# Wodlfvllf/QuintNet

Hardware: AMD Instinct MI355X
Metric: samples/sec (higher is better)
Workload: dtype bf16; 1 GPU; model=gpt2-124M, global_batch=32, seq_len=1024, micro_batch=32, grad_acc=1, parallelism=dp1_tp1_pp1, optimizer=zero1-adamw

## Files before the change

quintnet_amd/csrc/bindings.cpp:

```cpp
#include <torch/extension.h>
#include <ATen/cuda/CUDAContext.h>
#include <hip/hip_runtime.h>

#include <vector>

template <typename T>
void layernorm_fwd_launch(const T*, const T*, const T*, const T*, T*, T*, float*, float*, int, int, float, hipStream_t);
template <typename T>
void layernorm_bwd_launch(const T*, const T*, const T*, const float*, const float*, const T*, T*, float*, float*, int, int, hipStream_t);
int layernorm_bwd_chunks(int rows);
template <typename T>
void softmax_fwd_launch(const T*, T*, long long, int, int, float, int, hipStream_t);
template <typename T>
void softmax_bwd_launch(const T*, const T*, T*, long long, int, float, hipStream_t);
template <typename T>
void ce_fwd_launch(const T*, const long long*, float*, float*, long long, int, long long, hipStream_t);
template <typename T>
void ce_bwd_launch(const T*, const long long*, const float*, const float*, const long long*, T*, long long, int, long long, float, hipStream_t);
template <typename T>
void act_bwd_launch(const T*, const T*, T*, long long, int, hipStream_t);
template <typename T>
void colsum_launch(const T*, float*, long long, int, hipStream_t);
long long colsum_bf16_chunks(long long rows, int N);
int wgrad_tn_splits(int M, int N, int K);
void wgrad_tn_launch(const unsigned short*, const unsigned short*, float*,
                     unsigned short*, int, int, int, int, hipStream_t);
bool colsum_bf16_launch(const unsigned short*, float*, unsigned short*,
                        long long, int, hipStream_t);
template <typename T>
void dropout_fwd_launch(const T*, T*, unsigned char*, long long, float, unsigned, hipStream_t);
template <typename T>
void dropout_bwd_launch(const T*, T*, const unsigned char*, long long, float, hipStream_t);
template <typename T>
void embedding_pair_fwd_launch(const long long*, const T*, const T*, T*, long long, int, int, hipStream_t);
template <typename T>
void embedding_pair_bwd_launch(const long long*, const long long*, const T*, float*, float*, float*, long long, long long, int, int, hipStream_t);
long long embedding_bwd_chunks(long long rows);
template <typename TP, typename TG>
void adamw_launch(TP*, float*, const TG*, float*, float*, const long long*, long long, float, float, float, float, float, int, hipStream_t);
template <typename T>
void sumsq_launch(const T*, long long, float*, hipStream_t);
long long sumsq_blocks(long long n);
std::vector<at::Tensor> gemm_bias_gelu_aux(at::Tensor x, at::Tensor w,
                                           at::Tensor bias);
void gemm_nt_launch(const unsigned short*, const unsigned short*, const unsigned short*,
                    unsigned short*, unsigned short*, int, int, int, int, hipStream_t,
                    int mode = 0);
struct AttnStrides {
  long long qB, qH, qT, kB, kH, kT, vB, vH, vT, oB, oH, oT;
};
void attn_fwd_launch(const unsigned short*, const unsigned short*, const unsigned short*,
                     unsigned short*, float*, int, int, int, int, int, float,
                     int, const AttnStrides&, hipStream_t);
void attn_delta_launch(const unsigned short*, const unsigned short*, float*, int, int, int,
                       long long, long long, long long, long long, long long, long long,
                       hipStream_t);
void attn_bwd_dq_launch(const unsigned short*, const unsigned short*, const unsigned short*,
                        const unsigned short*, const float*, const float*, unsigned short*,
                        int, int, int, int, int, float, int, const AttnStrides&,
                        long long, long long, long long, hipStream_t);
void attn_bwd_dkv_launch(const unsigned short*, const unsigned short*, const unsigned short*,
                         const unsigned short*, const float*, const float*, unsigned short*,
                         unsigned short*, int, int, int, int, int, float, int, const AttnStrides&,
                         long long, long long, long long, long long, long long, long long,
                         long long, long long, long long, hipStream_t);

namespace {

hipStream_t cur_stream() {
  return (hipStream_t)at::cuda::getCurrentCUDAStream().stream();
}

const unsigned short* bf16p(const torch::Tensor& t) {
  return reinterpret_cast<const unsigned short*>(t.data_ptr<at::BFloat16>());
}
unsigned short* bf16p_mut(torch::Tensor& t) {
  return reinterpret_cast<unsigned short*>(t.data_ptr<at::BFloat16>());
}

#define CHECK_GPU(t) TORCH_CHECK(t.is_cuda(), #t " must be on GPU")

std::vector<torch::Tensor> gemm_nt(torch::Tensor x, torch::Tensor w,
                                   c10::optional<torch::Tensor> bias, int64_t act,
                                   int64_t mode) {
  CHECK_GPU(x); CHECK_GPU(w);
  TORCH_CHECK(x.dtype() == torch::kBFloat16 && w.dtype() == torch::kBFloat16,
              "gemm_nt: bf16 only");
  TORCH_CHECK(x.dim() == 2 && w.dim() == 2 && x.size(1) == w.size(1),
              "gemm_nt: shape mismatch");
  TORCH_CHECK(x.size(1) % 8 == 0, "gemm_nt: K must be a multiple of 8");
  auto xc = x.contiguous();
  auto wc = w.contiguous();
  int64_t M = xc.size(0), K = xc.size(1), N = wc.size(0);
  auto out = torch::empty({M, N}, xc.options());
  torch::Tensor pre;
  unsigned short* prep = nullptr;
  if (act != 0) {
    pre = torch::empty({M, N}, xc.options());
    prep = bf16p_mut(pre);
  }
  const unsigned short* bp = nullptr;
  torch::Tensor bc;
  if (bias.has_value() && bias->defined()) {
    bc = bias->contiguous();
    TORCH_CHECK(bc.dtype() == torch::kBFloat16, "bias must be bf16");
    bp = bf16p(bc);
  }
  gemm_nt_launch(bf16p(xc), bf16p(wc), bp, bf16p_mut(out), prep,
                 (int)M, (int)N, (int)K, (int)act, cur_stream(), (int)mode);
  if (act != 0) return {out, pre};
  return {out};
}

std::vector<torch::Tensor> layernorm_fwd(torch::Tensor x, torch::Tensor w,
                                         torch::Tensor b, double eps,
                                         c10::optional<torch::Tensor> residual) {
  CHECK_GPU(x);
  auto xc = x.contiguous();
  int64_t H = xc.size(-1);
  int64_t rows = xc.numel() / H;
  auto y = torch::empty_like(xc);
  auto mean = torch::empty({rows}, xc.options().dtype(torch::kFloat32));
  auto rstd = torch::empty({rows}, xc.options().dtype(torch::kFloat32));
  auto wc = w.contiguous(); auto bc = b.contiguous();
  torch::Tensor rc, sum_out;
  bool has_res = residual.has_value() && residual->defined();
  if (has_res) {
    rc = residual->contiguous();
    sum_out = torch::empty_like(xc);
  }
  if (xc.dtype() == torch::kBFloat16) {
    layernorm_fwd_launch<unsigned short>(
        bf16p(xc), has_res ? bf16p(rc) : nullptr, bf16p(wc), bf16p(bc),
        bf16p_mut(y), has_res ? bf16p_mut(sum_out) : nullptr,
        mean.data_ptr<float>(), rstd.data_ptr<float>(), (int)rows, (int)H,
        (float)eps, cur_stream());
  } else {
    layernorm_fwd_launch<float>(
        xc.data_ptr<float>(), has_res ? rc.data_ptr<float>() : nullptr,
        wc.data_ptr<float>(), bc.data_ptr<float>(), y.data_ptr<float>(),
        has_res ? sum_out.data_ptr<float>() : nullptr, mean.data_ptr<float>(),
        rstd.data_ptr<float>(), (int)rows, (int)H, (float)eps, cur_stream());
  }
  if (has_res) return {y, mean, rstd, sum_out};
  return {y, mean, rstd};
}

std::vector<torch::Tensor> layernorm_bwd(torch::Tensor dy, torch::Tensor x,
                                         torch::Tensor w, torch::Tensor mean,
                                         torch::Tensor rstd,
                                         c10::optional<torch::Tensor> dsum) {
  CHECK_GPU(x);
  auto dyc = dy.contiguous(); auto xc = x.contiguous(); auto wc = w.contiguous();
  int64_t H = xc.size(-1);
  int64_t rows = xc.numel() / H;
  auto dx = torch::empty_like(xc);
  int64_t chunks = layernorm_bwd_chunks((int)rows);
  auto part = torch::empty({2, chunks, H}, xc.options().dtype(torch::kFloat32));
  float* dwp = part.data_ptr<float>();
  float* dbp = dwp + chunks * H;
  torch::Tensor dsc;
  bool has_ds = dsum.has_value() && dsum->defined();
  if (has_ds) dsc = dsum->contiguous();
  if (xc.dtype() == torch::kBFloat16) {
    layernorm_bwd_launch<unsigned short>(
        bf16p(dyc), bf16p(xc), bf16p(wc), mean.data_ptr<float>(),
        rstd.data_ptr<float>(), has_ds ? bf16p(dsc) : nullptr, bf16p_mut(dx),
        dwp, dbp, (int)rows, (int)H, cur_stream());
  } else {
    layernorm_bwd_launch<float>(
        dyc.data_ptr<float>(), xc.data_ptr<float>(), wc.data_ptr<float>(),
        mean.data_ptr<float>(), rstd.data_ptr<float>(),
        has_ds ? dsc.data_ptr<float>() : nullptr, dx.data_ptr<float>(),
        dwp, dbp, (int)rows, (int)H, cur_stream());
  }
  auto dwdb = part.sum(1).to(w.dtype());
  return {dx, dwdb[0], dwdb[1]};
}

torch::Tensor softmax_fwd(torch::Tensor scores, double scale, bool causal) {
  CHECK_GPU(scores);
  auto sc = scores.contiguous();
  int64_t S = sc.size(-1);
  int64_t Tq = sc.size(-2);
  long long rows = sc.numel() / S;
  auto out = torch::empty_like(sc);
  if (sc.dtype() == torch::kBFloat16) {
    softmax_fwd_launch<unsigned short>(bf16p(sc), bf16p_mut(out), rows, (int)Tq,
                                       (int)S, (float)scale, causal ? 1 : 0,
                                       cur_stream());
  } else {
    softmax_fwd_launch<float>(sc.data_ptr<float>(), out.data_ptr<float>(), rows,
                              (int)Tq, (int)S, (float)scale, causal ? 1 : 0,
                              cur_stream());
  }
  return out;
}

torch::Tensor softmax_bwd(torch::Tensor p, torch::Tensor dp, double scale) {
  CHECK_GPU(p);
  auto pc = p.contiguous(); auto dpc = dp.contiguous();
  int64_t S = pc.size(-1);
  long long rows = pc.numel() / S;
  auto ds = torch::empty_like(pc);
  if (pc.dtype() == torch::kBFloat16) {
    softmax_bwd_launch<unsigned short>(bf16p(pc), bf16p(dpc), bf16p_mut(ds), rows,
                                       (int)S, (float)scale, cur_stream());
  } else {
    softmax_bwd_launch<float>(pc.data_ptr<float>(), dpc.data_ptr<float>(),
                              ds.data_ptr<float>(), rows, (int)S, (float)scale,
                              cur_stream());
  }
  return ds;
}

std::vector<torch::Tensor> cross_entropy_fwd(torch::Tensor logits,
                                             torch::Tensor target,
                                             int64_t ignore_index) {
  CHECK_GPU(logits);
  auto lc = logits.contiguous();
  auto tc = target.contiguous();
  TORCH_CHECK(tc.dtype() == torch::kInt64, "target must be int64");
  int64_t V = lc.size(-1);
  long long rows = lc.numel() / V;
  auto lse = torch::empty({(int64_t)rows}, lc.options().dtype(torch::kFloat32));
  auto row_loss = torch::empty({(int64_t)rows}, lc.options().dtype(torch::kFloat32));
  if (lc.dtype() == torch::kBFloat16) {
    ce_fwd_launch<unsigned short>(bf16p(lc), (const long long*)tc.data_ptr<int64_t>(),
                                  lse.data_ptr<float>(), row_loss.data_ptr<float>(),
                                  rows, (int)V, ignore_index, cur_stream());
  } else {
    ce_fwd_launch<float>(lc.data_ptr<float>(), (const long long*)tc.data_ptr<int64_t>(),
                         lse.data_ptr<float>(), row_loss.data_ptr<float>(), rows,
                         (int)V, ignore_index, cur_stream());
  }
  auto loss_sum = row_loss.sum();
  auto n_valid = (tc != ignore_index).sum();
  return {loss_sum, n_valid, lse};
}

torch::Tensor cross_entropy_bwd(torch::Tensor logits, torch::Tensor target,
                                torch::Tensor lse, torch::Tensor n_valid,
                                int64_t ignore_index,
                                c10::optional<torch::Tensor> grad_scale) {
  CHECK_GPU(logits);
  auto lc = logits.contiguous();
  auto tc = target.contiguous();
  int64_t V = lc.size(-1);
  long long rows = lc.numel() / V;
  auto dl = torch::empty_like(lc);
  auto nv = n_valid.to(torch::kInt64).contiguous();
  TORCH_CHECK(nv.is_cuda() && nv.numel() == 1, "n_valid must be a GPU scalar");
  const long long* nvp = (const long long*)nv.data_ptr<int64_t>();
  float inv_n = 1.0f;
  const float* gp = nullptr;
  torch::Tensor gs;
  if (grad_scale.has_value() && grad_scale->defined()) {
    gs = grad_scale->to(torch::kFloat32).contiguous();
    TORCH_CHECK(gs.numel() == 1, "grad_scale must be a scalar tensor");
    gp = gs.data_ptr<float>();
  }
  if (lc.dtype() == torch::kBFloat16) {
    ce_bwd_launch<unsigned short>(bf16p(lc), (const long long*)tc.data_ptr<int64_t>(),
                                  lse.data_ptr<float>(), gp, nvp, bf16p_mut(dl),
                                  rows, (int)V, ignore_index, inv_n, cur_stream());
  } else {
    ce_bwd_launch<float>(lc.data_ptr<float>(), (const long long*)tc.data_ptr<int64_t>(),
                         lse.data_ptr<float>(), gp, nvp, dl.data_ptr<float>(),
                         rows, (int)V, ignore_index, inv_n, cur_stream());
  }
  return dl;
}

torch::Tensor embedding_pair_fwd(torch::Tensor ids, torch::Tensor wte,
                                 torch::Tensor wpe) {
  CHECK_GPU(ids);
  auto ic = ids.contiguous();
  TORCH_CHECK(ic.dtype() == torch::kInt64, "ids must be int64");
  int64_t Tlen = ic.size(-1);
  long long rows = ic.numel();
  int64_t H = wte.size(1);
  auto out = torch::empty({ic.size(0), Tlen, H}, wte.options());
  if (wte.dtype() == torch::kBFloat16)
    embedding_pair_fwd_launch<unsigned short>(
        (const long long*)ic.data_ptr<int64_t>(), bf16p(wte), bf16p(wpe),
        bf16p_mut(out), rows, (int)Tlen, (int)H, cur_stream());
  else
    embedding_pair_fwd_launch<float>(
        (const long long*)ic.data_ptr<int64_t>(), wte.data_ptr<float>(),
        wpe.data_ptr<float>(), out.data_ptr<float>(), rows, (int)Tlen, (int)H,
        cur_stream());
  return out;
}

std::vector<torch::Tensor> embedding_pair_bwd(torch::Tensor ids, torch::Tensor dout,
                                              int64_t vocab, int64_t n_pos) {
  CHECK_GPU(ids);
  auto ic = ids.contiguous();
  auto dc = dout.contiguous();
  int64_t Tlen = ic.size(-1);
  long long rows = ic.numel();
  int64_t H = dc.size(-1);
  auto dwte = torch::zeros({vocab, H}, dc.options().dtype(torch::kFloat32));
  auto dwpe = torch::zeros({n_pos, H}, dc.options().dtype(torch::kFloat32));
  TORCH_CHECK(n_pos >= Tlen, "sequence longer than the position table");
  TORCH_CHECK(dc.numel() == rows * H, "dout does not match ids");
  auto sorted = ic.reshape({-1}).sort(true, 0, false);
  auto sid = std::get<0>(sorted).contiguous();
  auto perm = std::get<1>(sorted).contiguous();
  auto part = torch::empty({(int64_t)embedding_bwd_chunks(rows), 2, H},
                           dc.options().dtype(torch::kFloat32));
  if (dc.dtype() == torch::kBFloat16)
    embedding_pair_bwd_launch<unsigned short>(
        (const long long*)sid.data_ptr<int64_t>(),
        (const long long*)perm.data_ptr<int64_t>(), bf16p(dc),
        dwte.data_ptr<float>(), dwpe.data_ptr<float>(), part.data_ptr<float>(),
        rows, (long long)vocab,
        (int)Tlen, (int)H, cur_stream());
  else
    embedding_pair_bwd_launch<float>(
        (const long long*)sid.data_ptr<int64_t>(),
        (const long long*)perm.data_ptr<int64_t>(), dc.data_ptr<float>(),
        dwte.data_ptr<float>(), dwpe.data_ptr<float>(), part.data_ptr<float>(),
        rows, (long long)vocab,
        (int)Tlen, (int)H, cur_stream());
  return {dwte.to(dout.dtype()), dwpe.to(dout.dtype())};
}

std::vector<torch::Tensor> dropout_fwd(torch::Tensor x, double p, int64_t seed) {
  CHECK_GPU(x);
  auto xc = x.contiguous();
  auto y = torch::empty_like(xc);
  auto mask = torch::empty({xc.numel()}, xc.options().dtype(torch::kUInt8));
  if (xc.dtype() == torch::kBFloat16)
    dropout_fwd_launch<unsigned short>(bf16p(xc), bf16p_mut(y), mask.data_ptr<unsigned char>(),
                                       xc.numel(), (float)p, (unsigned)seed, cur_stream());
  else
    dropout_fwd_launch<float>(xc.data_ptr<float>(), y.data_ptr<float>(), mask.data_ptr<unsigned char>(),
                              xc.numel(), (float)p, (unsigned)seed, cur_stream());
  return {y, mask};
}

torch::Tensor dropout_bwd(torch::Tensor dy, torch::Tensor mask, double p) {
  CHECK_GPU(dy);
  auto dyc = dy.contiguous();
  auto dx = torch::empty_like(dyc);
  if (dyc.dtype() == torch::kBFloat16)
    dropout_bwd_launch<unsigned short>(bf16p(dyc), bf16p_mut(dx), mask.data_ptr<unsigned char>(),
                                       dyc.numel(), (float)p, cur_stream());
  else
    dropout_bwd_launch<float>(dyc.data_ptr<float>(), dx.data_ptr<float>(), mask.data_ptr<unsigned char>(),
                              dyc.numel(), (float)p, cur_stream());
  return dx;
}

torch::Tensor wgrad_tn(torch::Tensor dy, torch::Tensor x) {
  CHECK_GPU(dy); CHECK_GPU(x);
  TORCH_CHECK(dy.dtype() == torch::kBFloat16 && x.dtype() == torch::kBFloat16,
              "wgrad_tn: bf16 only");
  auto dyc = dy.contiguous(); auto xc = x.contiguous();
  TORCH_CHECK(dyc.dim() == 2 && xc.dim() == 2 && dyc.size(0) == xc.size(0),
              "wgrad_tn: [M,N],[M,K] expected");
  int64_t M = dyc.size(0), N = dyc.size(1), K = xc.size(1);
  TORCH_CHECK(N % 128 == 0 && K % 128 == 0 && M % 64 == 0,
              "wgrad_tn: shape not eligible");
  int splits = wgrad_tn_splits((int)M, (int)N, (int)K);
  auto slab = torch::empty({splits, N, K}, dyc.options().dtype(torch::kFloat32));
  auto out = torch::empty({N, K}, dyc.options());
  wgrad_tn_launch(bf16p(dyc), bf16p(xc), slab.data_ptr<float>(), bf16p_mut(out),
                  (int)M, (int)N, (int)K, splits, cur_stream());
  return out;
}

torch::Tensor colsum(torch::Tensor x) {
  CHECK_GPU(x);
  auto xc = x.contiguous();
  int64_t N = xc.size(-1);
  long long rows = xc.numel() / N;
  if (xc.dtype() == torch::kBFloat16 && (N & 7) == 0) {
    long long chunks = colsum_bf16_chunks(rows, (int)N);
    auto part = torch::empty({chunks, N}, xc.options().dtype(torch::kFloat32));
    auto out = torch::empty({N}, xc.options());
    if (colsum_bf16_launch(bf16p(xc), part.data_ptr<float>(), bf16p_mut(out),
                           rows, (int)N, cur_stream()))
      return out;
  }
  auto out = torch::zeros({N}, xc.options().dtype(torch::kFloat32));
  if (xc.dtype() == torch::kBFloat16)
    colsum_launch<unsigned short>(bf16p(xc), out.data_ptr<float>(), rows, (int)N, cur_stream());
  else
    colsum_launch<float>(xc.data_ptr<float>(), out.data_ptr<float>(), rows, (int)N, cur_stream());
  return out.to(x.dtype());
}

torch::Tensor act_bwd(torch::Tensor dy, torch::Tensor pre, int64_t act) {
  CHECK_GPU(dy);
  auto dyc = dy.contiguous();
  auto prec = pre.contiguous();
  TORCH_CHECK(dyc.numel() == prec.numel(), "act_bwd size mismatch");
  auto dx = torch::empty_like(dyc);
  if (dyc.dtype() == torch::kBFloat16)
    act_bwd_launch<unsigned short>(bf16p(dyc), bf16p(prec), bf16p_mut(dx),
                                   dyc.numel(), (int)act, cur_stream());
  else
    act_bwd_launch<float>(dyc.data_ptr<float>(), prec.data_ptr<float>(),
                          dx.data_ptr<float>(), dyc.numel(), (int)act, cur_stream());
  return dx;
}

void adamw_step(torch::Tensor param, torch::Tensor master, torch::Tensor grad,
                torch::Tensor m, torch::Tensor v, int64_t step, double lr,
                double beta1, double beta2, double eps, double wd,
                c10::optional<torch::Tensor> step_dev) {
  CHECK_GPU(param);
  long long n = param.numel();
  TORCH_CHECK(master.numel() == n && grad.numel() == n && m.numel() == n && v.numel() == n,
              "adamw_step: size mismatch");
  auto st = cur_stream();
  float* mp = master.data_ptr<float>();
  float* m1 = m.data_ptr<float>();
  float* m2 = v.data_ptr<float>();
  const long long* sd = nullptr;
  if (step_dev.has_value() && step_dev->defined())
    sd = (const long long*)step_dev->data_ptr<int64_t>();
  bool pbf = param.dtype() == torch::kBFloat16;
  bool gbf = grad.dtype() == torch::kBFloat16;
  if (pbf && gbf)
    adamw_launch<unsigned short, unsigned short>(bf16p_mut(param), mp, bf16p(grad), m1, m2, sd, n,
        (float)lr, (float)beta1, (float)beta2, (float)eps, (float)wd, (int)step, st);
  else if (pbf && !gbf)
    adamw_launch<unsigned short, float>(bf16p_mut(param), mp, grad.data_ptr<float>(), m1, m2, sd, n,
        (float)lr, (float)beta1, (float)beta2, (float)eps, (float)wd, (int)step, st);
  else if (!pbf && gbf)
    adamw_launch<float, unsigned short>(param.data_ptr<float>(), mp, bf16p(grad), m1, m2, sd, n,
        (float)lr, (float)beta1, (float)beta2, (float)eps, (float)wd, (int)step, st);
  else
    adamw_launch<float, float>(param.data_ptr<float>(), mp, grad.data_ptr<float>(), m1, m2, sd, n,
        (float)lr, (float)beta1, (float)beta2, (float)eps, (float)wd, (int)step, st);
}

torch::Tensor multi_tensor_sumsq(std::vector<torch::Tensor> tensors) {
  TORCH_CHECK(!tensors.empty(), "empty tensor list");
  int64_t total = 0;
  for (auto& t : tensors) total += sumsq_blocks(t.numel());
  auto part = torch::empty({total}, tensors[0].options().dtype(torch::kFloat32));
  auto st = cur_stream();
  int64_t off = 0;
  for (auto& t : tensors) {
    auto tc = t.contiguous();
    float* pp = part.data_ptr<float>() + off;
    if (tc.dtype() == torch::kBFloat16)
      sumsq_launch<unsigned short>(bf16p(tc), tc.numel(), pp, st);
    else
      sumsq_launch<float>(tc.data_ptr<float>(), tc.numel(), pp, st);
    off += sumsq_blocks(tc.numel());
  }
  return part.sum();
}


namespace {
void check_attn_view(const torch::Tensor& t, int64_t B, int64_t H, int64_t T) {
  TORCH_CHECK(t.dim() == 4 && t.size(0) == B && t.size(1) == H && t.size(2) == T &&
              t.size(3) == 64, "attn: bad view shape");
  TORCH_CHECK(t.stride(3) == 1, "attn: head_dim must be contiguous");
  TORCH_CHECK(t.stride(2) % 8 == 0 && t.stride(1) % 8 == 0 && t.stride(0) % 8 == 0,
              "attn: strides must be 16B-aligned");
  TORCH_CHECK(t.dtype() == torch::kBFloat16, "attn: bf16 only");
}
const unsigned short* ap(const torch::Tensor& t) {
  return reinterpret_cast<const unsigned short*>(t.data_ptr<at::BFloat16>());
}
unsigned short* ap_mut(torch::Tensor& t) {
  return reinterpret_cast<unsigned short*>(t.data_ptr<at::BFloat16>());
}
}

torch::Tensor attn_fwd(torch::Tensor q, torch::Tensor k, torch::Tensor v,
                       torch::Tensor out, double scale, bool causal,
                       int64_t q_offset) {
  int64_t B = q.size(0), H = q.size(1), Tq = q.size(2), Tk = k.size(2);
  TORCH_CHECK(Tq % 128 == 0 && Tk % 128 == 0 && q_offset % 128 == 0,
              "attn: Tq/Tk/q_offset must be multiples of 128");
  TORCH_CHECK(q_offset >= 0 && q_offset + Tq <= Tk,
              "attn: q rows [q_offset, q_offset+Tq) must lie within [0, Tk)");
  check_attn_view(q, B, H, Tq); check_attn_view(k, B, H, Tk);
  check_attn_view(v, B, H, Tk); check_attn_view(out, B, H, Tq);
  auto lse2 = torch::empty({B * H, Tq}, q.options().dtype(torch::kFloat32));
  AttnStrides st{q.stride(0), q.stride(1), q.stride(2), k.stride(0), k.stride(1),
                 k.stride(2), v.stride(0), v.stride(1), v.stride(2), out.stride(0),
                 out.stride(1), out.stride(2)};
  attn_fwd_launch(ap(q), ap(k), ap(v), ap_mut(out), lse2.data_ptr<float>(),
                  (int)B, (int)H, (int)Tq, (int)Tk, (int)q_offset, (float)scale,
                  causal ? 1 : 0, st, cur_stream());
  return lse2;
}

void attn_bwd(torch::Tensor q, torch::Tensor k, torch::Tensor v,
              torch::Tensor out, torch::Tensor dout, torch::Tensor lse2,
              torch::Tensor dq, torch::Tensor dk, torch::Tensor dv,
              double scale, bool causal, int64_t q_offset) {
  int64_t B = q.size(0), H = q.size(1), Tq = q.size(2), Tk = k.size(2);
  check_attn_view(dout, B, H, Tq); check_attn_view(dq, B, H, Tq);
  check_attn_view(dk, B, H, Tk); check_attn_view(dv, B, H, Tk);
  auto delta = torch::empty({B * H, Tq}, q.options().dtype(torch::kFloat32));
  attn_delta_launch(ap(dout), ap(out), delta.data_ptr<float>(), (int)B, (int)H,
                    (int)Tq, dout.stride(0), dout.stride(1), dout.stride(2),
                    out.stride(0), out.stride(1), out.stride(2), cur_stream());
  AttnStrides st{q.stride(0), q.stride(1), q.stride(2), k.stride(0), k.stride(1),
                 k.stride(2), v.stride(0), v.stride(1), v.stride(2), dq.stride(0),
                 dq.stride(1), dq.stride(2)};
  attn_bwd_dq_launch(ap(q), ap(k), ap(v), ap(dout), lse2.data_ptr<float>(),
                     delta.data_ptr<float>(), ap_mut(dq), (int)B, (int)H,
                     (int)Tq, (int)Tk, (int)q_offset,
                     (float)scale, causal ? 1 : 0, st, dout.stride(0),
                     dout.stride(1), dout.stride(2), cur_stream());
  attn_bwd_dkv_launch(ap(q), ap(k), ap(v), ap(dout), lse2.data_ptr<float>(),
                      delta.data_ptr<float>(), ap_mut(dk), ap_mut(dv), (int)B,
                      (int)H, (int)Tq, (int)Tk, (int)q_offset, (float)scale,
                      causal ? 1 : 0, st,
                      dout.stride(0), dout.stride(1), dout.stride(2),
                      dk.stride(0), dk.stride(1), dk.stride(2), dv.stride(0),
                      dv.stride(1), dv.stride(2), cur_stream());
}

}

PYBIND11_MODULE(TORCH_EXTENSION_NAME, m) {
  m.def("gemm_nt", &gemm_nt, "bf16 MFMA NT GEMM with fused bias/activation",
        py::arg("x"), py::arg("w"), py::arg("bias") = c10::nullopt,
        py::arg("act") = 0, py::arg("mode") = 0);
  m.def("layernorm_fwd", &layernorm_fwd);
  m.def("layernorm_bwd", &layernorm_bwd);
  m.def("softmax_fwd", &softmax_fwd);
  m.def("softmax_bwd", &softmax_bwd);
  m.def("cross_entropy_fwd", &cross_entropy_fwd);
  m.def("cross_entropy_bwd", &cross_entropy_bwd);
  m.def("act_bwd", &act_bwd, "fused activation backward");
  m.def("colsum", &colsum, "column sum (bias grad)");
  m.def("wgrad_tn", &wgrad_tn, "split-K TN weight gradient (tr-read MFMA)");
  m.def("dropout_fwd", &dropout_fwd);
  m.def("embedding_pair_fwd", &embedding_pair_fwd);
  m.def("embedding_pair_bwd", &embedding_pair_bwd);
  m.def("dropout_bwd", &dropout_bwd);
  m.def("attn_fwd", &attn_fwd, "fused flash attention forward (D=64)",
        py::arg("q"), py::arg("k"), py::arg("v"), py::arg("out"),
        py::arg("scale"), py::arg("causal"), py::arg("q_offset") = 0);
  m.def("attn_bwd", &attn_bwd, "fused flash attention backward (D=64)",
        py::arg("q"), py::arg("k"), py::arg("v"), py::arg("out"),
        py::arg("dout"), py::arg("lse2"), py::arg("dq"), py::arg("dk"),
        py::arg("dv"), py::arg("scale"), py::arg("causal"),
        py::arg("q_offset") = 0);
  m.def("adamw_step", &adamw_step);
  m.def("gemm_bias_gelu_aux", &gemm_bias_gelu_aux,
        "hipBLASLt GEMM + fused bias/GELU epilogue (aux = pre-activation)");
  m.def("multi_tensor_sumsq", &multi_tensor_sumsq);
  m.attr("gfx") = "gfx950";
}
```

quintnet_amd/csrc/layernorm.hip:

```cpp
#include "common.h"

template <typename T, int WPB>
__global__ void layernorm_fwd_kernel(
    const T* __restrict__ x, const T* __restrict__ res,
    const T* __restrict__ w, const T* __restrict__ b,
    T* __restrict__ y, T* __restrict__ sum_out,
    float* __restrict__ mean_out, float* __restrict__ rstd_out,
    int rows, int H, float eps) {
  const int lane = threadIdx.x & (QN_WAVE - 1);
  const int wave = threadIdx.x / QN_WAVE;
  const long long row = (long long)blockIdx.x * WPB + wave;
  if (row >= rows) return;
  const T* xr = x + row * H;
  const T* rr = res ? res + row * H : nullptr;
  T* yr = y + row * H;
  T* sr = sum_out ? sum_out + row * H : nullptr;

  float sum = 0.f, sq = 0.f;
  float cache[16];
  const bool cached = H <= QN_WAVE * 16;
  const bool vec8 = sizeof(T) == 2 && (H & 7) == 0 && H >= 512;
  if (cached && vec8) {
    int n = 0;
    for (int i = lane * 8; i < H; i += QN_WAVE * 8, n += 8) {
      ld8_f32(reinterpret_cast<const unsigned short*>(xr) + i, cache + n);
      if (rr) {
        float rv[8];
        ld8_f32(reinterpret_cast<const unsigned short*>(rr) + i, rv);
#pragma unroll
        for (int j = 0; j < 8; ++j) cache[n + j] += rv[j];
        if (sr) st8_f32(reinterpret_cast<unsigned short*>(sr) + i, cache + n);
      }
#pragma unroll
      for (int j = 0; j < 8; ++j) {
        sum += cache[n + j];
        sq += cache[n + j] * cache[n + j];
      }
    }
  } else if (cached) {
    int n = 0;
    for (int i = lane; i < H; i += QN_WAVE, ++n) {
      float f = ld_as_f32(xr + i);
      if (rr) {
        f += ld_as_f32(rr + i);
        if (sr) st_from_f32(sr + i, f);
      }
      cache[n] = f;
      sum += f; sq += f * f;
    }
  } else {
    for (int i = lane; i < H; i += QN_WAVE) {
      float f = ld_as_f32(xr + i);
      if (rr) {
        f += ld_as_f32(rr + i);
        if (sr) st_from_f32(sr + i, f);
      }
      sum += f; sq += f * f;
    }
  }
  sum = wave_reduce_sum(sum);
  sq = wave_reduce_sum(sq);
  const float mean = sum / H;
  const float var = fmaxf(sq / H - mean * mean, 0.f);
  const float rstd = rsqrtf(var + eps);
  if (lane == 0) { mean_out[row] = mean; rstd_out[row] = rstd; }

  if (cached && vec8) {
    int n = 0;
    for (int i = lane * 8; i < H; i += QN_WAVE * 8, n += 8) {
      float wv[8], bv[8], ov[8];
      ld8_f32(reinterpret_cast<const unsigned short*>(w) + i, wv);
      ld8_f32(reinterpret_cast<const unsigned short*>(b) + i, bv);
#pragma unroll
      for (int j = 0; j < 8; ++j)
        ov[j] = (cache[n + j] - mean) * rstd * wv[j] + bv[j];
      st8_f32(reinterpret_cast<unsigned short*>(yr) + i, ov);
    }
  } else if (cached) {
    int n = 0;
    for (int i = lane; i < H; i += QN_WAVE, ++n) {
      float wi = ld_as_f32(w + i);
      float bi = ld_as_f32(b + i);
      st_from_f32(yr + i, (cache[n] - mean) * rstd * wi + bi);
    }
  } else {
    for (int i = lane; i < H; i += QN_WAVE) {
      float f = ld_as_f32(xr + i);
      if (rr) f += ld_as_f32(rr + i);
      float wi = ld_as_f32(w + i);
      float bi = ld_as_f32(b + i);
      st_from_f32(yr + i, (f - mean) * rstd * wi + bi);
    }
  }
}

template <typename T, int WPB>
__global__ void layernorm_bwd_dx_kernel(
    const T* __restrict__ dy, const T* __restrict__ x, const T* __restrict__ w,
    const float* __restrict__ mean_in, const float* __restrict__ rstd_in,
    const T* __restrict__ dsum, T* __restrict__ dx, int rows, int H) {
  const int lane = threadIdx.x & (QN_WAVE - 1);
  const int wave = threadIdx.x / QN_WAVE;
  const long long row = (long long)blockIdx.x * WPB + wave;
  if (row >= rows) return;
  const T* xr = x + row * H;
  const T* dyr = dy + row * H;
  const T* dsr = dsum ? dsum + row * H : nullptr;
  T* dxr = dx + row * H;
  const float mean = mean_in[row], rstd = rstd_in[row];

  float cx[16], cwdy[16];
  const bool cached = H <= QN_WAVE * 16;
  const bool vec8 = sizeof(T) == 2 && (H & 7) == 0 && H >= 512;
  float c1 = 0.f, c2 = 0.f;
  if (cached && vec8) {
    int n = 0;
    for (int i = lane * 8; i < H; i += QN_WAVE * 8, n += 8) {
      float xv[8], wv[8], dv[8];
      ld8_f32(reinterpret_cast<const unsigned short*>(xr) + i, xv);
      ld8_f32(reinterpret_cast<const unsigned short*>(w) + i, wv);
      ld8_f32(reinterpret_cast<const unsigned short*>(dyr) + i, dv);
#pragma unroll
      for (int j = 0; j < 8; ++j) {
        float xhat = (xv[j] - mean) * rstd;
        float wdy = wv[j] * dv[j];
        cx[n + j] = xhat; cwdy[n + j] = wdy;
        c1 += wdy; c2 += wdy * xhat;
      }
    }
  } else if (cached) {
    int n = 0;
    for (int i = lane; i < H; i += QN_WAVE, ++n) {
      float xhat = (ld_as_f32(xr + i) - mean) * rstd;
      float wdy = ld_as_f32(w + i) * ld_as_f32(dyr + i);
      cx[n] = xhat; cwdy[n] = wdy;
      c1 += wdy; c2 += wdy * xhat;
    }
  } else {
    for (int i = lane; i < H; i += QN_WAVE) {
      float xhat = (ld_as_f32(xr + i) - mean) * rstd;
      float wdy = ld_as_f32(w + i) * ld_as_f32(dyr + i);
      c1 += wdy; c2 += wdy * xhat;
    }
  }
  c1 = wave_reduce_sum(c1) / H;
  c2 = wave_reduce_sum(c2) / H;

  if (cached && vec8) {
    int n = 0;
    for (int i = lane * 8; i < H; i += QN_WAVE * 8, n += 8) {
      float ov[8];
#pragma unroll
      for (int j = 0; j < 8; ++j) ov[j] = (cwdy[n + j] - c1 - cx[n + j] * c2) * rstd;
      if (dsr) {
        float dsv[8];
        ld8_f32(reinterpret_cast<const unsigned short*>(dsr) + i, dsv);
#pragma unroll
        for (int j = 0; j < 8; ++j) ov[j] += dsv[j];
      }
      st8_f32(reinterpret_cast<unsigned short*>(dxr) + i, ov);
    }
  } else if (cached) {
    int n = 0;
    for (int i = lane; i < H; i += QN_WAVE, ++n) {
      float v = (cwdy[n] - c1 - cx[n] * c2) * rstd;
      if (dsr) v += ld_as_f32(dsr + i);
      st_from_f32(dxr + i, v);
    }
  } else {
    for (int i = lane; i < H; i += QN_WAVE) {
      float xhat = (ld_as_f32(xr + i) - mean) * rstd;
      float wdy = ld_as_f32(w + i) * ld_as_f32(dyr + i);
      float v = (wdy - c1 - xhat * c2) * rstd;
      if (dsr) v += ld_as_f32(dsr + i);
      st_from_f32(dxr + i, v);
    }
  }
}

template <typename T>
__global__ void layernorm_bwd_dwdb_kernel(
    const T* __restrict__ dy, const T* __restrict__ x,
    const float* __restrict__ mean_in, const float* __restrict__ rstd_in,
    float* __restrict__ dw, float* __restrict__ db, int rows, int H) {
  const int col = blockIdx.x * blockDim.x + threadIdx.x;
  if (col >= H) return;
  const int r0 = blockIdx.y;
  const int nchunks = gridDim.y;
  float aw = 0.f, ab = 0.f;
  for (long long r = r0; r < rows; r += nchunks) {
    float dyv = ld_as_f32(dy + r * H + col);
    float xhat = (ld_as_f32(x + r * H + col) - mean_in[r]) * rstd_in[r];
    aw += dyv * xhat;
    ab += dyv;
  }
  dw[(long long)r0 * H + col] = aw;
  db[(long long)r0 * H + col] = ab;
}

int layernorm_bwd_chunks(int rows) { return min(max(rows / 64, 1), 256); }

template <typename T>
void layernorm_fwd_launch(const T* x, const T* res, const T* w, const T* b,
                          T* y, T* sum_out, float* mean, float* rstd, int rows,
                          int H, float eps, hipStream_t stream) {
  constexpr int WPB = 4;
  dim3 grid((rows + WPB - 1) / WPB);
  hipLaunchKernelGGL((layernorm_fwd_kernel<T, WPB>), grid, dim3(WPB * QN_WAVE), 0,
                     stream, x, res, w, b, y, sum_out, mean, rstd, rows, H, eps);
}

template <typename T>
void layernorm_bwd_launch(const T* dy, const T* x, const T* w, const float* mean,
                          const float* rstd, const T* dsum, T* dx, float* dw,
                          float* db, int rows, int H, hipStream_t stream) {
  constexpr int WPB = 4;
  dim3 grid((rows + WPB - 1) / WPB);
  hipLaunchKernelGGL((layernorm_bwd_dx_kernel<T, WPB>), grid, dim3(WPB * QN_WAVE),
                     0, stream, dy, x, w, mean, rstd, dsum, dx, rows, H);
  int colblocks = (H + 255) / 256;
  int chunks = layernorm_bwd_chunks(rows);
  hipLaunchKernelGGL((layernorm_bwd_dwdb_kernel<T>), dim3(colblocks, chunks),
                     dim3(256), 0, stream, dy, x, mean, rstd, dw, db, rows, H);
}

template void layernorm_fwd_launch<float>(const float*, const float*, const float*, const float*,
                                          float*, float*, float*, float*, int, int, float, hipStream_t);
template void layernorm_fwd_launch<unsigned short>(const unsigned short*, const unsigned short*,
                                                   const unsigned short*, const unsigned short*,
                                                   unsigned short*, unsigned short*, float*,
                                                   float*, int, int, float, hipStream_t);
template void layernorm_bwd_launch<float>(const float*, const float*, const float*, const float*,
                                          const float*, const float*, float*, float*, float*, int, int, hipStream_t);
template void layernorm_bwd_launch<unsigned short>(const unsigned short*, const unsigned short*,
                                                   const unsigned short*, const float*, const float*,
                                                   const unsigned short*, unsigned short*, float*, float*, int, int, hipStream_t);
```

Before: 680.4 samples/s.

## Fuse LayerNorm backward dx and dw/db partial sums into one-pass kernel

Adds a bf16 LayerNorm backward kernel that computes dx and the per-chunk dw/db partial sums in a single pass. Each block owns a row chunk, stages xhat and dy in shared memory, and prefetches the next row's data into registers. This removes the second kernel that re-read x and dy from global memory to compute the weight and bias gradients. The kernel uses about 96KB of shared memory per block and only 256 blocks, which may limit occupancy and parallelism.

```diff
diff --git a/quintnet_amd/csrc/bindings.cpp b/quintnet_amd/csrc/bindings.cpp
--- a/quintnet_amd/csrc/bindings.cpp
+++ b/quintnet_amd/csrc/bindings.cpp
@@ -9,6 +9,11 @@
 template <typename T>
 void layernorm_bwd_launch(const T*, const T*, const T*, const float*, const float*, const T*, T*, float*, float*, int, int, hipStream_t);
 int layernorm_bwd_chunks(int rows);
+bool layernorm_bwd_fused_shape_ok(int H);
+void layernorm_bwd_fused_launch(const unsigned short*, const unsigned short*,
+                                const unsigned short*, const float*, const float*,
+                                const unsigned short*, unsigned short*, float*,
+                                float*, int, int, hipStream_t);
 template <typename T>
 void softmax_fwd_launch(const T*, T*, long long, int, int, float, int, hipStream_t);
 template <typename T>
@@ -146,6 +151,8 @@
   return {y, mean, rstd};
 }
 
+bool aligned16(const void* p) { return ((uintptr_t)p & 15u) == 0; }
+
 std::vector<torch::Tensor> layernorm_bwd(torch::Tensor dy, torch::Tensor x,
                                          torch::Tensor w, torch::Tensor mean,
                                          torch::Tensor rstd,
@@ -154,15 +161,29 @@
   auto dyc = dy.contiguous(); auto xc = x.contiguous(); auto wc = w.contiguous();
   int64_t H = xc.size(-1);
   int64_t rows = xc.numel() / H;
+  TORCH_CHECK(dyc.numel() == xc.numel() && wc.numel() == H &&
+                  mean.numel() == rows && rstd.numel() == rows,
+              "layernorm_bwd: shape mismatch");
   auto dx = torch::empty_like(xc);
+  torch::Tensor dsc;
+  bool has_ds = dsum.has_value() && dsum->defined();
+  if (has_ds) {
+    dsc = dsum->contiguous();
+    TORCH_CHECK(dsc.numel() == xc.numel(), "layernorm_bwd: dsum shape mismatch");
+  }
   int64_t chunks = layernorm_bwd_chunks((int)rows);
   auto part = torch::empty({2, chunks, H}, xc.options().dtype(torch::kFloat32));
   float* dwp = part.data_ptr<float>();
   float* dbp = dwp + chunks * H;
-  torch::Tensor dsc;
-  bool has_ds = dsum.has_value() && dsum->defined();
-  if (has_ds) dsc = dsum->contiguous();
-  if (xc.dtype() == torch::kBFloat16) {
+  if (xc.dtype() == torch::kBFloat16 && wc.dtype() == torch::kBFloat16 &&
+      layernorm_bwd_fused_shape_ok((int)H) && aligned16(xc.data_ptr()) &&
+      aligned16(dyc.data_ptr()) && aligned16(wc.data_ptr()) &&
+      aligned16(dx.data_ptr()) && (!has_ds || aligned16(dsc.data_ptr()))) {
+    layernorm_bwd_fused_launch(
+        bf16p(dyc), bf16p(xc), bf16p(wc), mean.data_ptr<float>(),
+        rstd.data_ptr<float>(), has_ds ? bf16p(dsc) : nullptr, bf16p_mut(dx),
+        dwp, dbp, (int)rows, (int)H, cur_stream());
+  } else if (xc.dtype() == torch::kBFloat16) {
     layernorm_bwd_launch<unsigned short>(
         bf16p(dyc), bf16p(xc), bf16p(wc), mean.data_ptr<float>(),
         rstd.data_ptr<float>(), has_ds ? bf16p(dsc) : nullptr, bf16p_mut(dx),
@@ -532,6 +553,9 @@
         py::arg("act") = 0, py::arg("mode") = 0);
   m.def("layernorm_fwd", &layernorm_fwd);
   m.def("layernorm_bwd", &layernorm_bwd);
+  m.def("layernorm_bwd_chunks", [](int64_t rows) {
+    return (int64_t)layernorm_bwd_chunks((int)rows);
+  }, "row chunks (= blocks of the one-pass kernel) LayerNorm backward uses");
   m.def("softmax_fwd", &softmax_fwd);
   m.def("softmax_bwd", &softmax_bwd);
   m.def("cross_entropy_fwd", &cross_entropy_fwd);
diff --git a/quintnet_amd/csrc/layernorm.hip b/quintnet_amd/csrc/layernorm.hip
--- a/quintnet_amd/csrc/layernorm.hip
+++ b/quintnet_amd/csrc/layernorm.hip
@@ -200,6 +200,134 @@
 
 int layernorm_bwd_chunks(int rows) { return min(max(rows / 64, 1), 256); }
 
+constexpr int LNF_WPB = 16;
+constexpr int LNF_MAXH = 1024;
+
+__global__ void __launch_bounds__(LNF_WPB * QN_WAVE)
+layernorm_bwd_fused_kernel(
+    const unsigned short* __restrict__ dy, const unsigned short* __restrict__ x,
+    const unsigned short* __restrict__ w, const float* __restrict__ mean_in,
+    const float* __restrict__ rstd_in, const unsigned short* __restrict__ dsum,
+    unsigned short* __restrict__ dx, float* __restrict__ dw,
+    float* __restrict__ db, int rows, int H) {
+#pragma clang fp contract(off)
+  __shared__ float s_xhat[LNF_WPB][LNF_MAXH];
+  __shared__ __attribute__((aligned(16))) unsigned short s_dy[LNF_WPB][LNF_MAXH];
+  const int lane = threadIdx.x & (QN_WAVE - 1);
+  const int wave = threadIdx.x / QN_WAVE;
+  const int nchunks = gridDim.x;
+  const int chunk = blockIdx.x;
+  const int nk = chunk < rows ? (rows - chunk + nchunks - 1) / nchunks : 0;
+  const int i0 = lane * 8, i1 = lane * 8 + QN_WAVE * 8;
+
+  float aw = 0.f, ab = 0.f;
+  s16x8 xq[2] = {{0}, {0}}, dq[2] = {{0}, {0}};
+  if (wave < nk) {
+    const long long off = ((long long)chunk + (long long)wave * nchunks) * H;
+    if (i0 < H) {
+      xq[0] = *reinterpret_cast<const s16x8*>(x + off + i0);
+      dq[0] = *reinterpret_cast<const s16x8*>(dy + off + i0);
+    }
+    if (i1 < H) {
+      xq[1] = *reinterpret_cast<const s16x8*>(x + off + i1);
+      dq[1] = *reinterpret_cast<const s16x8*>(dy + off + i1);
+    }
+  }
+
+  for (int k0 = 0; k0 < nk; k0 += LNF_WPB) {
+    const int k = k0 + wave;
+    s16x8 xn[2] = {xq[0], xq[1]}, dn[2] = {dq[0], dq[1]};
+    if (k + LNF_WPB < nk) {
+      const long long off =
+          ((long long)chunk + (long long)(k + LNF_WPB) * nchunks) * H;
+      if (i0 < H) {
+        xn[0] = *reinterpret_cast<const s16x8*>(x + off + i0);
+        dn[0] = *reinterpret_cast<const s16x8*>(dy + off + i0);
+      }
+      if (i1 < H) {
+        xn[1] = *reinterpret_cast<const s16x8*>(x + off + i1);
+        dn[1] = *reinterpret_cast<const s16x8*>(dy + off + i1);
+      }
+    }
+    if (k < nk) {
+      const long long row = (long long)chunk + (long long)k * nchunks;
+      const unsigned short* dsr = dsum ? dsum + row * H : nullptr;
+      unsigned short* dxr = dx + row * H;
+      const float mean = mean_in[row], rstd = rstd_in[row];
+
+      float cx[16], cwdy[16];
+      float c1 = 0.f, c2 = 0.f;
+#pragma unroll
+      for (int kk = 0; kk < 2; ++kk) {
+        const int i = kk == 0 ? i0 : i1;
+        if (i < H) {
+          float wv[8];
+          ld8_f32(w + i, wv);
+#pragma unroll
+          for (int j = 0; j < 8; ++j) {
+            float xhat = (bf16_to_f32((unsigned short)xq[kk][j]) - mean) * rstd;
+            float wdy = wv[j] * bf16_to_f32((unsigned short)dq[kk][j]);
+            cx[kk * 8 + j] = xhat; cwdy[kk * 8 + j] = wdy;
+            c1 += wdy;
+            c2 = j == 0 ? __builtin_fmaf(wdy, xhat, c2) : c2 + wdy * xhat;
+            s_xhat[wave][i + j] = xhat;
+          }
+          *reinterpret_cast<s16x8*>(&s_dy[wave][i]) = dq[kk];
+        }
+      }
+      c1 = wave_reduce_sum(c1) / H;
+      c2 = wave_reduce_sum(c2) / H;
+
+#pragma unroll
+      for (int kk = 0; kk < 2; ++kk) {
+        const int i = kk == 0 ? i0 : i1;
+        if (i < H) {
+          float ov[8];
+#pragma unroll
+          for (int j = 0; j < 8; ++j)
+            ov[j] = __builtin_fmaf(-cx[kk * 8 + j], c2, cwdy[kk * 8 + j] - c1) * rstd;
+          if (dsr) {
+            float dsv[8];
+            ld8_f32(dsr + i, dsv);
+#pragma unroll
+            for (int j = 0; j < 8; ++j) ov[j] += dsv[j];
+          }
+          st8_f32(dxr + i, ov);
+        }
+      }
+    }
+    __syncthreads();
+    const int nact = min(LNF_WPB, nk - k0);
+    if ((int)threadIdx.x < H) {
+      for (int r = 0; r < nact; ++r) {
+        const float d = bf16_to_f32(s_dy[r][threadIdx.x]);
+        aw = aw + s_xhat[r][threadIdx.x] * d;
+        ab = ab + d;
+      }
+    }
+    __syncthreads();
+    xq[0] = xn[0]; xq[1] = xn[1]; dq[0] = dn[0]; dq[1] = dn[1];
+  }
+  if ((int)threadIdx.x < H) {
+    dw[(long long)chunk * H + threadIdx.x] = aw;
+    db[(long long)chunk * H + threadIdx.x] = ab;
+  }
+}
+
+bool layernorm_bwd_fused_shape_ok(int H) {
+  return (H & 7) == 0 && H >= 512 && H <= LNF_MAXH;
+}
+
+void layernorm_bwd_fused_launch(const unsigned short* dy, const unsigned short* x,
+                                const unsigned short* w, const float* mean,
+                                const float* rstd, const unsigned short* dsum,
+                                unsigned short* dx, float* dw, float* db,
+                                int rows, int H, hipStream_t stream) {
+  hipLaunchKernelGGL(layernorm_bwd_fused_kernel, dim3(layernorm_bwd_chunks(rows)),
+                     dim3(LNF_WPB * QN_WAVE), 0, stream, dy, x, w, mean, rstd,
+                     dsum, dx, dw, db, rows, H);
+}
+
 template <typename T>
 void layernorm_fwd_launch(const T* x, const T* res, const T* w, const T* b,
                           T* y, T* sum_out, float* mean, float* rstd, int rows,
```

Result: faster. 692.5 samples/s (median of 6 runs) (+1.8%).
